# usnistgov/object-detection-yolov3

Measured on AMD Instinct MI355X. Metric: images/sec (train fwd+bwd) bs=8 416x416, higher is better.
Workload: dtype f32

## Files before the change

include/yolo3hip.h:

```cpp
#ifndef YOLO3HIP_H
#define YOLO3HIP_H

#include <math.h>
#include <stddef.h>
#include <stdint.h>

#ifdef __cplusplus
extern "C" {
#endif

#define Y3_OK 0
#define Y3_EINVAL (-1)
#define Y3_ELAUNCH (-2)

typedef void* y3_stream_t;

const char* y3_last_error(void);
int y3_debug_div(int x, int d);
int y3_version(void);

#define Y3_EPI_LRELU 1u
#define Y3_EPI_ACCUM 2u
#define Y3_CONV_X3 4u
int y3_x3_split_weights(const float* w, void* planes, int taps, int rows, int k_per_row, y3_stream_t stream);
int y3_x3_split_weights_batched(const float* arena, void* planes_arena, const int* table_dev, int nlayers, int total_blocks, y3_stream_t stream);
int y3_x3_prepare_weights_batched(const float* params, float* params_t, void* planes, void* planes_t, const int* table_dev, int nlayers,
                                  int total_tiles, y3_stream_t stream);

typedef struct y3_tensor {
    float* ptr;
    int n, h, w, c;
    int ld;
} y3_tensor;

int y3_conv2d_fwd(const y3_tensor* src, const float* wt, const float* bias, int ksize, int stride,
                  const y3_tensor* dst, unsigned flags, float alpha,
                  const float* scale, const float* shift, const y3_tensor* resid,
                  float* stats, void* workspace, size_t workspace_bytes, y3_stream_t stream);
int y3_conv2d_stats_tiles(int m, int cin, int ksize, int cout);
size_t y3_conv2d_fwd_workspace(int m, int cin, int ksize, int cout);
int y3_conv2d_stats_tiles_x(int m, int cin, int ksize, int cout, unsigned flags);
size_t y3_conv2d_fwd_workspace_x(int m, int cin, int ksize, int cout, unsigned flags);
int y3_conv2d_x3_ok(int m, int c, int ntaps, int nout);
int y3_conv2d_dgrad_x3_ok(const y3_tensor* ddst, int ksize, int stride, const y3_tensor* dsrc);
size_t y3_conv2d_plan(int m, int cin, int ksize, int cout, int* out13);
size_t y3_conv2d_plan_x(int m, int cin, int ksize, int cout, unsigned flags, int* out13);

int y3_conv2d_dgrad(const y3_tensor* ddst, const float* wt_t, int ksize, int stride,
                    const y3_tensor* dsrc, unsigned flags, void* workspace, size_t workspace_bytes,
                    y3_stream_t stream);
size_t y3_conv2d_dgrad_workspace(const y3_tensor* ddst, int ksize, int stride, const y3_tensor* dsrc);
size_t y3_conv2d_dgrad_workspace_x(const y3_tensor* ddst, int ksize, int stride, const y3_tensor* dsrc, unsigned flags);
int y3_conv2d_dgrad_bn(const y3_tensor* ddst, const float* wt_t, int ksize, int stride, const y3_tensor* dsrc,
                       unsigned flags, const y3_tensor* bn_a, float* bn_partials,
                       void* workspace, size_t workspace_bytes, y3_stream_t stream);
int y3_conv2d_dgrad_bn_tiles(const y3_tensor* ddst, int ksize, int stride, const y3_tensor* dsrc);
int y3_conv2d_dgrad_bn_tiles_x(const y3_tensor* ddst, int ksize, int stride, const y3_tensor* dsrc, unsigned flags);
size_t y3_conv2d_dgrad_plan_x(const y3_tensor* ddst, int ksize, int stride, const y3_tensor* dsrc, unsigned flags, int* out51);

int y3_conv2d_wgrad(const y3_tensor* src, const y3_tensor* ddst, int ksize, int stride,
                    float* dw, void* workspace, size_t workspace_bytes, y3_stream_t stream);
size_t y3_conv2d_wgrad_workspace(const y3_tensor* src, const y3_tensor* ddst, int ksize, int stride);
int y3_conv2d_wgrad_x(const y3_tensor* src, const y3_tensor* ddst, int ksize, int stride,
                      float* dw, unsigned flags, void* workspace, size_t workspace_bytes, y3_stream_t stream);
size_t y3_conv2d_wgrad_workspace_x(const y3_tensor* src, const y3_tensor* ddst, int ksize, int stride, unsigned flags);
int y3_conv2d_wgrad_x3_ok(int m, int cin, int ksize, int cout);
size_t y3_conv2d_wgrad_plan(int m, int cin, int ksize, int cout, int* out8);
size_t y3_conv2d_wgrad_plan_x(int m, int cin, int ksize, int cout, unsigned flags, int* out8);

int y3_transpose_weights(const float* wt, float* wt_t, int taps, int cin, int cout, y3_stream_t stream);
int y3_transpose_weights_batched(const float* params, float* params_t, const int* table_dev, int nlayers,
                                 int total_tiles, y3_stream_t stream);

int y3_bn_stats_finalize(const float* stats, int tiles, int c, int count,
                         const float* gamma, const float* beta, float eps, float momentum,
                         float* moving_mean, float* moving_var,
                         float* save_mean, float* save_rstd, float* scale, float* shift,
                         y3_stream_t stream);
int y3_bn_fold_inference(const float* gamma, const float* beta, const float* moving_mean,
                         const float* moving_var, float eps, int c, float* scale, float* shift,
                         y3_stream_t stream);
int y3_bn_fold_inference_batched(const float* params, const float* moving, float* chan, const int* table_dev,
                                 int nlayers, float eps, y3_stream_t stream);
int y3_bn_apply(const y3_tensor* a, const float* scale, const float* shift, const y3_tensor* resid,
                const y3_tensor* y, y3_stream_t stream);
int y3_bn_bwd_stats(const y3_tensor* dy, const y3_tensor* a, const y3_tensor* dres, int dres_accumulate,
                    const float* gamma, const float* save_mean, const float* save_rstd, float alpha,
                    float* dgamma, float* dbeta, float* dbias, float* coef,
                    void* workspace, size_t workspace_bytes, y3_stream_t stream);
// ... 219 lines not shown
```

object-detection-yolov3_amd/csrc/conv.hip:

```cpp
#include <stdlib.h>

#include <type_traits>
#include <utility>

#include "common.h"
#include "conv_plan.h"

template <int BM, int BN, int WM, int WN, int BK>
__global__ __launch_bounds__(64 * WM * WN) void conv_igemm_kernel(const ConvArgs p) {
    constexpr int THREADS = 64 * WM * WN;
    constexpr int LDA = BK + 4;
    constexpr int TM = BM / WM, TN = BN / WN, MB = TM / 32, NB = TN / 32;
    constexpr int KV = BK / 4;
    constexpr int A_TOTAL = BM * KV, A_LOADS = (A_TOTAL + THREADS - 1) / THREADS;
    constexpr int BN4 = BN / 4;
    constexpr int B_TOTAL = BK * BN4, B_LOADS = (B_TOTAL + THREADS - 1) / THREADS;
    static_assert(THREADS % KV == 0 && TM % 32 == 0 && TN % 32 == 0, "tile shape");

    __shared__ __attribute__((aligned(16))) float As[2][BM * LDA];
    __shared__ __attribute__((aligned(16))) float Bs[2][BK * BN];
    __shared__ float red[2][WM][BN];

    const int tid = threadIdx.x, lane = tid & 63, wave = tid >> 6;
    const int l31 = lane & 31, lh = lane >> 5;
// ... 1174 lines not shown
        for (int kw = 0; kw < ksize; ++kw) {
            const int t = kh * ksize + kw;
            p.tap_dhdw |= (unsigned long long)((kh - pbh + 1) | ((kw - pbw + 1) << 2)) << (4 * t);
        }
    p.src = src->ptr;
    p.ddst = ddst->ptr;
    p.H = src->h;
    p.W = src->w;
    p.C = src->c;
    p.src_ld = src->ld;
    p.OH = OH;
    p.OW = OW;
    p.sh = p.sw = stride;
    p.dd_ld = ddst->ld;
    p.Nout = ddst->c;
    p.K = taps * src->c;
    p.M = src->n * OH * OW;
    {
        const long long sb = (long long)src->n * src->h * src->w * src->ld * 4, db = (long long)p.M * ddst->ld * 4;
        Y3_CHECK_ARG(sb < 0x7fffffffLL && db < 0x7fffffffLL, "conv2d_wgrad: tensors of 2 GiB or more are not supported (32-bit buffer offsets)");
        p.src_bytes = (unsigned)sb;
        p.dd_bytes = (unsigned)db;
    }
    Y3_CHECK_ARG((flags & ~Y3_CONV_X3) == 0, "conv2d_wgrad: only Y3_CONV_X3 allowed in flags");
    const WgradPlan w = describe_wgrad(p.M, src->c, taps, p.Nout, flags);
    Y3_CHECK_ARG(!(flags & Y3_CONV_X3) || w.x3, "conv2d_wgrad: Y3_CONV_X3 does not take this shape (ask y3_conv2d_wgrad_x3_ok())");
    p.chunk = w.chunk;
    p.nbn = y3_cdiv(p.Nout, w.bn);
    p.ohw = OH * OW;
    p.ntaps = taps;
    p.dv_tiles = y3_make_div(w.tiles);
    p.dv_nbn = y3_make_div(p.nbn);
    p.dv_ohw = y3_make_div(p.ohw);
    p.dv_ow = y3_make_div(OW);
    const size_t need = w.ws_bytes;
    Y3_CHECK_ARG(workspace_bytes >= need && (need == 0 || workspace), "conv2d_wgrad: workspace %zu < %zu", workspace_bytes, need);
    Y3_CHECK_ARG(need < 0x7ff00000ull, "conv2d_wgrad: slab area too large (%zu bytes)", need);
    p.tickets = w.in_kernel ? (int*)workspace : nullptr;
    if (p.tickets)
        if (int e = check_tickets("conv2d_wgrad", workspace, (hipStream_t)stream)) return e;
    p.out = w.splits > 1 ? (float*)((char*)workspace + Y3_WS_HEADER) : dw;
    p.dw = dw;
    hipStream_t st = (hipStream_t)stream;
    p.tiles = w.tiles;
    p.splits = w.splits;
    dim3 grid((unsigned)w.grid);
    constexpr int pad40 = 8192;
    if (w.x3) {
// ... 41 lines not shown
```

object-detection-yolov3_amd/csrc/conv_plan.cpp:

```cpp
#include <stdlib.h>
#include "host.h"
#include "conv_plan.h"

static TileCfg pick_tile(int M, int Nout) {
    TileCfg t;
    if (Nout <= 32)
        t = {128, 32, 16};
    else if (Nout <= 64)
        t = {128, 64, 16};
    else {
        const long long t128 = (long long)y3_cdiv(M, 128) * y3_cdiv(Nout, 128);
        const long long t64x128 = (long long)y3_cdiv(M, 64) * y3_cdiv(Nout, 128);
        if (t128 >= 600)
            t = {128, 128, 16};
        else if (t64x128 >= 600)
            t = {64, 128, 16};
        else
            t = {64, 64, 16};
    }
    return t;
}
void whole_tiles(ConvPlan& pl, int chunk) {
    pl.f = pl.tiles;
    pl.s0 = pl.s1 = 1;
// ... 448 lines not shown
            w.bn = 64;
        } else if (K <= 576) {
            w.bkr = 64;
        }
    }
    w.tiles = y3_cdiv(K, w.bkr) * y3_cdiv(Nout, w.bn);
    constexpr int want_waves = 4096;
    const int waves_per_wg = (w.bkr == 64 && w.bn == 32) ? 2 : 4;
    int splits = y3_cdiv(want_waves, w.tiles * waves_per_wg);
    const int maxs = y3_cdiv(M, 128);
    if (splits > maxs) splits = maxs;
    if (splits < 1) splits = 1;
    if (splits < y3_cdiv(M, Y3_WG_TABLE - 32)) splits = y3_cdiv(M, Y3_WG_TABLE - 32);
    int chunk = y3_cdiv(M, splits);
    chunk = y3_cdiv(chunk, 32) * 32;
    w.splits = y3_cdiv(M, chunk);
    w.chunk = chunk;
    return w;
}

static bool wgrad_x3_shape_ok(int K, int Nout, int taps, int cin) {
    return cin % 4 == 0 && K >= 128 && Nout >= 128 && (taps == 1 || y3_is_pow2(cin));
}
static WgradPlan plan_wgrad_x3(int K, int Nout, int M) {
    WgradPlan w;
    w.bkr = 128;
    w.bn = 128;
    w.tiles = y3_cdiv(K, 128) * y3_cdiv(Nout, 128);
    constexpr int want = 480;
    int splits = want / w.tiles;
    if (splits < 1) splits = 1;
    if (w.tiles > 256 && splits < 3) splits = 3;
    const int maxs = y3_cdiv(M, 192);
    if (splits > maxs) splits = maxs;
    if (splits < y3_cdiv(M, Y3_WG_TABLE - 96)) splits = y3_cdiv(M, Y3_WG_TABLE - 96);
    int chunk = y3_cdiv(M, splits);
    chunk = y3_cdiv(chunk, 96) * 96;
    w.splits = y3_cdiv(M, chunk);
    w.chunk = chunk;
    return w;
}

static bool wgrad_in_kernel(const WgradPlan& w) {
    return w.splits > 1 && w.splits <= Y3_WG_FANIN && w.tiles <= Y3_MAX_TICKETS;
}
static size_t wgrad_ws_bytes(const WgradPlan& w, int K, int Nout) {
    if (w.splits <= 1) return 0;
    if (wgrad_in_kernel(w)) return (size_t)Y3_WS_HEADER + (size_t)w.tiles * w.splits * w.bkr * w.bn * sizeof(float);
    return (size_t)Y3_WS_HEADER + (size_t)w.splits * K * Nout * sizeof(float);
}
WgradPlan describe_wgrad(int M, int cin, int taps, int Nout, unsigned flags) {
    const bool x3 = (flags & Y3_CONV_X3) && wgrad_x3_shape_ok(taps * cin, Nout, taps, cin);
    WgradPlan w = x3 ? plan_wgrad_x3(taps * cin, Nout, M) : plan_wgrad(taps * cin, Nout, M, taps);
    w.x3 = x3;
    w.grid = (w.splits >= 32 ? y3_cdiv(w.splits, 8) * 8 : w.splits) * w.tiles;
    w.in_kernel = wgrad_in_kernel(w);
    w.ws_bytes = wgrad_ws_bytes(w, taps * cin, Nout);
    return w;
}

extern "C" size_t y3_conv2d_wgrad_plan(int m, int cin, int ksize, int cout, int* out8) { return y3_conv2d_wgrad_plan_x(m, cin, ksize, cout, 0u, out8); }
extern "C" size_t y3_conv2d_wgrad_plan_x(int m, int cin, int ksize, int cout, unsigned flags, int* out8) {
    const WgradPlan w = describe_wgrad(m, cin, ksize * ksize, cout, flags);
    if (out8) {
        const int v[8] = {w.bkr, w.bn, w.splits, w.chunk, w.tiles, w.in_kernel ? 1 : 0, w.grid, Y3_WG_TABLE};
        for (int i = 0; i < 8; ++i) out8[i] = v[i];
    }
    return w.ws_bytes;
}

extern "C" int y3_conv2d_wgrad_x3_ok(int m, int cin, int ksize, int cout) {
    return (m > 0 && wgrad_x3_shape_ok(ksize * ksize * cin, cout, ksize * ksize, cin)) ? 1 : 0;
}
extern "C" size_t y3_conv2d_wgrad_workspace_x(const y3_tensor* src, const y3_tensor* ddst, int ksize, int stride, unsigned flags) {
    (void)stride;
    return describe_wgrad(ddst->n * ddst->h * ddst->w, src->c, ksize * ksize, ddst->c, flags).ws_bytes;
}
extern "C" size_t y3_conv2d_wgrad_workspace(const y3_tensor* src, const y3_tensor* ddst, int ksize, int stride) {
    return y3_conv2d_wgrad_workspace_x(src, ddst, ksize, stride, 0u);
}
```

object-detection-yolov3_amd/csrc/conv_x3.hip:

```cpp
#include "conv_fast.h"

typedef __bf16 y3_bf16x8 __attribute__((ext_vector_type(8)));
typedef __bf16 y3_bf16x2 __attribute__((ext_vector_type(2)));
typedef float y3_f32x2 __attribute__((ext_vector_type(2)));

__device__ __forceinline__ unsigned x3_pk(float a, float b) {
    const y3_f32x2 v = {a, b};
    return __builtin_bit_cast(unsigned, __builtin_convertvector(v, y3_bf16x2));
}
__device__ __forceinline__ float x3_lo(unsigned pk) { return __uint_as_float(pk << 16); }
__device__ __forceinline__ float x3_hi(unsigned pk) { return __uint_as_float(pk & 0xffff0000u); }

#ifndef Y3_X3_GB
#define Y3_X3_GB 4
#endif

template <int BM, int BN, int WM, int WN, bool DENSE, bool BNS>
__device__ __forceinline__ void conv_x3_body(const FastArgs& p, const int braw, const int grid) {
    constexpr int BK = 16, KV = 4;
    constexpr int THREADS = 64 * WM * WN;
    constexpr int TM = BM / WM, TN = BN / WN, MB = TM / 32, NB = TN / 32;
    constexpr int A_LOADS = BM * KV / THREADS;
    constexpr int B_LOADS = BN * 6 / THREADS;
    static_assert((BM * KV) % THREADS == 0 && (BN * 6) % THREADS == 0 && TM % 32 == 0 && TN % 32 == 0, "tile shape");
// ... 579 lines not shown
}

template <int BM, int BN, int WM, int WN>
static void x3_launch_tile(const FastArgs& p, bool dense, int grid, hipStream_t st) {
    const dim3 g(grid), b(64 * WM * WN);
    if (p.bn_a)
        hipLaunchKernelGGL((conv_x3_kernel<BM, BN, WM, WN, true, true>), g, b, 0, st, p);
    else if (dense)
        hipLaunchKernelGGL((conv_x3_kernel<BM, BN, WM, WN, true, false>), g, b, 0, st, p);
    else
        hipLaunchKernelGGL((conv_x3_kernel<BM, BN, WM, WN, false, false>), g, b, 0, st, p);
}

typedef short y3_s16x4 __attribute__((ext_vector_type(4)));

__device__ __forceinline__ y3_bf16x8 x3_tr_pair(const unsigned short* a0, const unsigned short* a1) {
    const y3_s16x4 lo = __builtin_amdgcn_ds_read_tr16_b64_v4i16((y3_s16x4 __attribute__((address_space(3)))*)(a0));
    const y3_s16x4 hi = __builtin_amdgcn_ds_read_tr16_b64_v4i16((y3_s16x4 __attribute__((address_space(3)))*)(a1));
    typedef short s16x8 __attribute__((ext_vector_type(8)));
    const s16x8 v = {lo[0], lo[1], lo[2], lo[3], hi[0], hi[1], hi[2], hi[3]};
    return __builtin_bit_cast(y3_bf16x8, v);
}

template <int BKR, int BN, int WM, int WN>
__global__ __launch_bounds__(64 * WM * WN, 2) void conv_wgrad_x3_kernel(const WgradArgs p) {
    constexpr int BP = 16;
    constexpr int THREADS = 64 * WM * WN;
    constexpr int TM = BKR / WM, TN = BN / WN, MB = TM / 32, NB = TN / 32;
    constexpr int KR4 = BKR / 4, BN4 = BN / 4;
    static_assert(BKR == 128 && BN == 128 && THREADS == 256, "the swizzled [16][128] images and the loader are written for 128 x 128 tiles");
    constexpr int A_LOADS = BP * KR4 / THREADS, B_LOADS = BP * BN4 / THREADS;
    constexpr int PSTEP = THREADS / KR4;
    constexpr int PLANE = BP * 128;
    constexpr int OPB = 3 * PLANE;
    constexpr int BUF = 2 * OPB;
    __shared__ __attribute__((aligned(16))) unsigned short lds[2 * BUF];
    __shared__ uint2 pix[Y3_WG_TABLE];

    const int tid = threadIdx.x, lane = tid & 63, wave = tid >> 6;
    const int wm = wave / WN, wn = wave % WN;
    int splits = p.splits, tiles = p.tiles, nbn = p.nbn, chunk = p.chunk, aM = p.M, ohw = p.ohw, OW = p.OW, aH = p.H, aW = p.W;
    int src_ld = p.src_ld, csh = p.sh, csw = p.sw, ntaps = p.ntaps;
    unsigned dt_m = p.dv_tiles.mul, dn_m = p.dv_nbn.mul, dohw_m = p.dv_ohw.mul, dow_m = p.dv_ow.mul;
    int dt_s = p.dv_tiles.shift, dn_s = p.dv_nbn.shift, dohw_s = p.dv_ohw.shift, dow_s = p.dv_ow.shift;
    unsigned dhdw_lo = (unsigned)p.tap_dhdw, dhdw_hi = (unsigned)(p.tap_dhdw >> 32);
    Y3_PIN_S(splits); Y3_PIN_S(tiles); Y3_PIN_S(nbn); Y3_PIN_S(chunk); Y3_PIN_S(aM); Y3_PIN_S(ohw); Y3_PIN_S(OW); Y3_PIN_S(aH); Y3_PIN_S(aW);
    Y3_PIN_S(src_ld); Y3_PIN_S(csh); Y3_PIN_S(csw); Y3_PIN_S(ntaps);
    Y3_PIN_S(dt_m); Y3_PIN_S(dn_m); Y3_PIN_S(dohw_m); Y3_PIN_S(dow_m); Y3_PIN_S(dt_s); Y3_PIN_S(dn_s); Y3_PIN_S(dohw_s); Y3_PIN_S(dow_s);
    Y3_PIN_S(dhdw_lo); Y3_PIN_S(dhdw_hi);
    const Y3Div dv_tiles = {dt_m, dt_s}, dv_nbn = {dn_m, dn_s}, dv_ohw = {dohw_m, dohw_s}, dv_ow = {dow_m, dow_s};
    const unsigned long long tap_dhdw = ((unsigned long long)dhdw_hi << 32) | dhdw_lo;
    int split, bid;
    if (splits >= 32) {
        const int xcd = blockIdx.x & 7, jx = blockIdx.x >> 3;
        const int q = y3_div(jx, dv_tiles);
        split = q * 8 + xcd;
        bid = jx - q * tiles;
    } else {
// ... 17 lines not shown
                const int oh = y3_div(r, dv_ow), ow = r - oh * OW;
                const int ih0 = oh * csh, iw0 = ow * csw;
                off = (unsigned)(((n * aH + ih0) * aW + iw0) * src_ld) * 4u;
                for (int t = 0; t < ntaps; ++t) {
                    const int code = (int)((tap_dhdw >> (4 * t)) & 15ull);
                    const int ih = ih0 + (code & 3) - 1, iw = iw0 + (code >> 2) - 1;
                    if ((unsigned)ih < (unsigned)aH && (unsigned)iw < (unsigned)aW) msk |= 1u << t;
                }
            }
            pix[pl] = make_uint2(off, msk);
        }
    }
    const __amdgpu_buffer_rsrc_t rs_src = __builtin_amdgcn_make_buffer_rsrc(const_cast<float*>(p.src), 0, p.src_bytes, 0x00020000);
    const __amdgpu_buffer_rsrc_t rs_dd = __builtin_amdgcn_make_buffer_rsrc(const_cast<float*>(p.ddst), 0, p.dd_bytes, 0x00020000);
    const int a_kv = tid % KR4;
    const int ak = k0 + a_kv * 4;
    const bool ak_ok = ak < p.K;
    const int atap = ak_ok ? (ak >> p.logC) : 0;
    const int ac = ak & p.cmask;
    const int acode = (int)((tap_dhdw >> (4 * atap)) & 15ull);
    const int a_tapoff = ((((acode & 3) - 1) * p.W + ((acode >> 2) - 1)) * p.src_ld + ac) * 4;
    const unsigned a_bit = ak_ok ? 1u << atap : 0u;
    const int pp0 = tid / KR4;
    const int bnn = n0 + a_kv * 4;
    const bool bn_ok = bnn < p.Nout;
    const unsigned b_lane = (unsigned)(bnn * 4);
    auto swz = [](int row) { return ((row & 3) << 2) | ((row >> 2) & 3); };
    int st_off[A_LOADS];
#pragma unroll
    for (int i = 0; i < A_LOADS; ++i) {
        const int row = pp0 + i * PSTEP;
        st_off[i] = row * 128 + 8 * ((a_kv >> 1) ^ swz(row)) + 4 * (a_kv & 1);
    }
    int fr_a[MB][2], fr_b[NB][2];
    {
        const int g = lane >> 4, li = lane & 15, q = li >> 2, pc = li & 3, h = g >> 1;
#pragma unroll
        for (int j = 0; j < 2; ++j) {
            const int row = 8 * h + 4 * j + q;
#pragma unroll
            for (int i = 0; i < MB; ++i) {
                const int c = wm * TM + i * 32 + 16 * (g & 1) + 4 * pc;
                fr_a[i][j] = row * 128 + 8 * ((c >> 3) ^ swz(row)) + (c & 4);
            }
#pragma unroll
            for (int i = 0; i < NB; ++i) {
                const int c = wn * TN + i * 32 + 16 * (g & 1) + 4 * pc;
                fr_b[i][j] = row * 128 + 8 * ((c >> 3) ^ swz(row)) + (c & 4);
            }
        }
    }

    f32x4 ra[3][A_LOADS], rb[3][B_LOADS];
    uint2 pe[A_LOADS];
    auto tload = [&](int step) {
#pragma unroll
        for (int i = 0; i < A_LOADS; ++i) pe[i] = pix[step * BP + pp0 + i * PSTEP];
    };
    auto gload_a = [&](auto I, int step, auto S) {
        constexpr int i = decltype(I)::value;
        const bool ok = ((pe[i].y & a_bit) != 0) & (step < nsteps);
        ra[decltype(S)::value][i] = __builtin_amdgcn_raw_buffer_load_b128(rs_src, ok ? pe[i].x + (unsigned)a_tapoff : Y3_OOB, 0, 0);
    };
    auto gload_b = [&](auto I, int step, auto S) {
        constexpr int i = decltype(I)::value;
        const int m = mbeg + step * BP + pp0 + i * PSTEP;
        const bool ok = (m < mend) & bn_ok;
        rb[decltype(S)::value][i] = __builtin_amdgcn_raw_buffer_load_b128(rs_dd, ok ? (unsigned)(m * p.dd_ld) * 4u + b_lane : Y3_OOB, 0, 0);
    };
    X3Pk pk = {0, 0};
    auto sub = [&](auto S, auto E, int buf) {
        constexpr int set = decltype(S)::value, e = decltype(E)::value, w = e / 4, sb = e % 4;
        if constexpr (w < A_LOADS) {
            unsigned short* d = &lds[buf * BUF + st_off[w]];
            x3_split_sub<sb>(ra[set][w], pk, d, d + PLANE, d + 2 * PLANE);
        } else {
            unsigned short* d = &lds[buf * BUF + OPB + st_off[w - A_LOADS]];
            x3_split_sub<sb>(rb[set][w - A_LOADS], pk, d, d + PLANE, d + 2 * PLANE);
        }
    };
    y3_bf16x8 FA[2][3][MB], FB[2][3][NB];
    auto read_a = [&](auto F, auto PC, int i, int buf) {
        const unsigned short* b = &lds[buf * BUF + decltype(PC)::value * PLANE];
        FA[decltype(F)::value][decltype(PC)::value][i] = x3_tr_pair(b + fr_a[i][0], b + fr_a[i][1]);
    };
    auto read_b = [&](auto F, auto PC, int j, int buf) {
        const unsigned short* b = &lds[buf * BUF + OPB + decltype(PC)::value * PLANE];
        FB[decltype(F)::value][decltype(PC)::value][j] = x3_tr_pair(b + fr_b[j][0], b + fr_b[j][1]);
    };

    f32x16 acc[MB][NB];
#pragma unroll
    for (int i = 0; i < MB; ++i)
#pragma unroll
        for (int j = 0; j < NB; ++j)
#pragma unroll
            for (int r = 0; r < 16; ++r) acc[i][j][r] = 0.f;

    using C0 = std::integral_constant<int, 0>;
    using C1 = std::integral_constant<int, 1>;
    using C2 = std::integral_constant<int, 2>;
    constexpr int NW = A_LOADS + B_LOADS;
    __syncthreads();
    if (nsteps > 0) {
        constexpr int NMG = MB * NB, NM = 6 * NMG, SB = Y3_X3_GB * NMG, SP = NM - SB;
        constexpr int NR1 = NB + MB + MB, NS = NW * 4;
        constexpr int NR2 = MB + NB + NB, RS2 = (NR2 + 1) / 2;
        static_assert(NR1 <= SB && RS2 + (NW + 1) / 2 + 1 <= SP, "not enough MFMA slots for the events of a step");
        auto step = [&](auto U, int s6) {
            constexpr int u = decltype(U)::value, cur = u & 1;
            using F = std::integral_constant<int, cur>;
            using G = std::integral_constant<int, cur ^ 1>;
            using RS = std::integral_constant<int, (u + 1) % 3>;
            const int st = s6 + u;
            y3_for_each_ic(std::make_integer_sequence<int, NM>{}, [&](auto Mi) {
                constexpr int m = decltype(Mi)::value;
                constexpr int g = m / NMG, i = (m % NMG) / NB, j = m % NB;
                constexpr int pa = g < 3 ? 0 : (g < 5 ? 1 : 2), pb = g < 3 ? g : (g == 3 ? 0 : (g == 4 ? 1 : 0));
                if constexpr (m == SB) {
                    y3_lds_barrier();
                    __builtin_amdgcn_sched_barrier(0);
                }
                acc[i][j] = __builtin_amdgcn_mfma_f32_32x32x16_bf16(FA[cur][pa][i], FB[cur][pb][j], acc[i][j], 0, 0, 0);
                __builtin_amdgcn_sched_barrier(0);
                if constexpr (m < SB) {
                    if constexpr (m < NB)
                        read_b(F{}, C2{}, m, cur);
                    else if constexpr (m < NB + MB)
// ... 96 lines not shown
#pragma unroll
                    for (int r = 0; r < 4; ++r) {
                        const f32x4 v = __builtin_amdgcn_raw_buffer_load_b128(rs_slab, base2, (unsigned)(((i * NB + j) * 4 + r) * THREADS * 16), 16 );
#pragma unroll
                        for (int e = 0; e < 4; ++e) acc[i][j][4 * r + e] = z == 0 ? v[e] : acc[i][j][4 * r + e] + v[e];
                    }
        }
    }
    float* out = p.tickets != nullptr ? p.dw : p.out + (p.splits > 1 ? (long long)split * p.K * p.Nout : 0ll);
#pragma unroll
    for (int j = 0; j < NB; ++j) {
        const int n = n0 + wn * TN + j * 32 + l31;
#pragma unroll
        for (int i = 0; i < MB; ++i)
#pragma unroll
            for (int r = 0; r < 16; ++r) {
                const int k = k0 + wm * TM + i * 32 + (r & 3) + 8 * (r >> 2) + 4 * lh;
                if (k < p.K && n < p.Nout) out[(long long)k * p.Nout + n] = acc[i][j][r];
            }
    }
}

bool y3_wgrad_x3_launch(const WgradArgs& p, int bkr, int bn, unsigned grid, hipStream_t st) {
    if (bkr != 128 || bn != 128) return false;
    hipLaunchKernelGGL((conv_wgrad_x3_kernel<128, 128, 2, 2>), dim3(grid), dim3(256), 0, st, p);
    return true;
}

__device__ __forceinline__ void x3_split_store(const float* __restrict__ w, unsigned short* __restrict__ planes, long long e, int rows, int C) {
    const long long tr = e / C;
    const int c = (int)(e - tr * C);
    const long long tap = tr / rows;
    const int row = (int)(tr - tap * rows);
    f32x4 r = *reinterpret_cast<const f32x4*>(w + e);
    const unsigned a0 = x3_pk(r[0], r[1]), a1 = x3_pk(r[2], r[3]);
    r[0] -= x3_lo(a0); r[1] -= x3_hi(a0); r[2] -= x3_lo(a1); r[3] -= x3_hi(a1);
    const unsigned b0 = x3_pk(r[0], r[1]), b1 = x3_pk(r[2], r[3]);
    r[0] -= x3_lo(b0); r[1] -= x3_hi(b0); r[2] -= x3_lo(b1); r[3] -= x3_hi(b1);
    unsigned short* d = planes + (((tap * (C >> 4) + (c >> 4)) * rows + row) * 3) * 16 + (c & 15);
    *reinterpret_cast<uint2*>(d) = make_uint2(a0, a1);
    *reinterpret_cast<uint2*>(d + 16) = make_uint2(b0, b1);
    *reinterpret_cast<uint2*>(d + 32) = make_uint2(x3_pk(r[0], r[1]), x3_pk(r[2], r[3]));
}
__global__ __launch_bounds__(256) void x3_split_weights_kernel(const float* __restrict__ w, unsigned short* __restrict__ planes, long long count, int rows, int C) {
    const long long e = ((long long)blockIdx.x * 256 + threadIdx.x) * 4;
    if (e < count) x3_split_store(w, planes, e, rows, C);
}
__global__ __launch_bounds__(256) void x3_split_weights_batched_kernel(const float* __restrict__ arena, unsigned short* __restrict__ planes_arena,
// ... 126 lines not shown
```

object-detection-yolov3_amd/yolo3/_hip.py:

```python
import ctypes as C
import os

import torch

_HERE = os.path.dirname(os.path.abspath(__file__))
LIB_PATH = os.environ.get('Y3_LIB') or os.path.join(_HERE, '_lib', 'libyolo3hip.so')


class HipLibraryMissing(ImportError):
    pass


class HipError(RuntimeError):
    pass


if not os.path.exists(LIB_PATH):
    raise HipLibraryMissing(
        'libyolo3hip.so not found at %s: build it with `make -C object-detection-yolov3_amd/csrc` '
        '(hipcc --offload-arch=gfx950).  There is no CPU fallback.' % LIB_PATH)

lib = C.CDLL(LIB_PATH)


# ... 10 lines not shown
    'y3_debug_div': (i32, [i32, i32]),
    'y3_version': (i32, []),
    'y3_conv2d_fwd': (i32, [TP, fp, fp, i32, i32, TP, u32, f32, fp, fp, TP, fp, vp, sz, vp]),
    'y3_conv2d_stats_tiles': (i32, [i32, i32, i32, i32]),
    'y3_conv2d_fwd_workspace': (sz, [i32, i32, i32, i32]),
    'y3_conv2d_dgrad': (i32, [TP, fp, i32, i32, TP, u32, vp, sz, vp]),
    'y3_conv2d_stats_tiles_x': (i32, [i32, i32, i32, i32, u32]),
    'y3_conv2d_fwd_workspace_x': (sz, [i32, i32, i32, i32, u32]),
    'y3_conv2d_x3_ok': (i32, [i32, i32, i32, i32]),
    'y3_conv2d_dgrad_x3_ok': (i32, [TP, i32, i32, TP]),
    'y3_x3_split_weights': (i32, [fp, vp, i32, i32, i32, vp]),
    'y3_x3_split_weights_batched': (i32, [fp, vp, ip, i32, i32, vp]),
    'y3_x3_prepare_weights_batched': (i32, [fp, fp, vp, vp, ip, i32, i32, vp]),
    'y3_conv2d_dgrad_workspace_x': (sz, [TP, i32, i32, TP, u32]),
    'y3_conv2d_dgrad_bn_tiles_x': (i32, [TP, i32, i32, TP, u32]),
    'y3_conv2d_dgrad_workspace': (sz, [TP, i32, i32, TP]),
    'y3_conv2d_dgrad_bn': (i32, [TP, fp, i32, i32, TP, u32, TP, fp, vp, sz, vp]),
    'y3_conv2d_dgrad_bn_tiles': (i32, [TP, i32, i32, TP]),
    'y3_conv2d_wgrad': (i32, [TP, TP, i32, i32, fp, vp, sz, vp]),
    'y3_conv2d_wgrad_workspace': (sz, [TP, TP, i32, i32]),
    'y3_conv2d_wgrad_x': (i32, [TP, TP, i32, i32, fp, u32, vp, sz, vp]),
    'y3_conv2d_wgrad_workspace_x': (sz, [TP, TP, i32, i32, u32]),
    'y3_conv2d_wgrad_x3_ok': (i32, [i32, i32, i32, i32]),
    'y3_transpose_weights': (i32, [fp, fp, i32, i32, i32, vp]),
    'y3_transpose_weights_batched': (i32, [fp, fp, ip, i32, i32, vp]),
    'y3_bn_stats_finalize': (i32, [fp, i32, i32, i32, fp, fp, f32, f32, fp, fp, fp, fp, fp, fp, vp]),
    'y3_bn_fold_inference': (i32, [fp, fp, fp, fp, f32, i32, fp, fp, vp]),
    'y3_bn_fold_inference_batched': (i32, [fp, fp, fp, ip, i32, f32, vp]),
    'y3_bn_apply': (i32, [TP, fp, fp, TP, TP, vp]),
    'y3_bn_bwd_stats': (i32, [TP, TP, TP, i32, fp, fp, fp, f32, fp, fp, fp, fp, vp, sz, vp]),
    'y3_bn_bwd_workspace': (sz, [i32, i32]),
    'y3_bn_bwd_apply': (i32, [TP, TP, fp, f32, TP, vp]),
    'y3_bn_bwd_apply_fanin': (i32, [TP, TP, fp, f32, TP, TP, i32, vp]),
    'y3_bn_bwd_finalize_tiles': (i32, [fp, i32, i32, i32, fp, fp, fp, f32, fp, fp, fp, fp, vp]),
    'y3_upsample_sum2x_fwd': (i32, [TP, TP, vp]),
    'y3_upsample_sum2x_bwd': (i32, [TP, TP, vp]),
    'y3_spp_fwd': (i32, [TP, TP, vp]),
    'y3_spp_fwd_bf16': (i32, [TP, TP, vp]),
    'y3_spp_bwd': (i32, [TP, TP, TP, i32, vp]),
    'y3_copy': (i32, [TP, TP, vp]),
    'y3_conv2d_fwd_bf16': (i32, [TP, vp, fp, i32, i32, TP, i32, u32, f32, fp, fp, TP, vp]),
    'y3_conv2d_fwd_bf16_ws': (i32, [TP, vp, fp, i32, i32, TP, i32, u32, f32, fp, fp, TP, vp, sz, vp]),
    'y3_conv2d_fwd_bf16_workspace': (sz, [i32, i32, i32, i32]),
    'y3_conv2d_fwd_bf16_plan': (sz, [TP, vp, fp, i32, i32, TP, i32, u32, f32, fp, fp, TP, vp, sz, ip]),
    'y3_f32_to_bf16': (i32, [fp, vp, sz, vp]),
    'y3_conv2d_first_bf16': (i32, [TP, fp, fp, TP, u32, f32, fp, fp, vp]),
# ... 53 lines not shown
    'y3_mosaic_batch': (i32, [fp, i32, i32, i32, i32, vp, fp, vp]),
    'y3_format_labels': (i32, [ip, ip, i32, i32, C.POINTER(C.c_float), i32, i32, i32, i32, fp, fp, fp, vp]),
    'y3_eval_offsets':(i32, [ip, i32, i32, i32, ip, vp]),
    'y3_eval_match': (i32, [fp, i32, i32, i32, i32, f32, f32, ip, ip, fp, i32, i32, fp, ip, i32, i32, C.POINTER(C.c_float), i32, ip,
                            vp, vp, C.c_longlong, vp]),
    'y3_eval_ap': (i32, [vp, vp, C.c_longlong, i32, i32, ip, vp, sz, fp, fp, ip, ip, vp]),
    'y3_eval_ap_workspace_bytes': (sz, [C.c_longlong, i32]),
    'y3_eval_match_ranges': (i32, [fp, i32, i32, i32, i32, f32, f32, ip, ip, fp, i32, i32, fp, ip, i32, i32, C.POINTER(C.c_float), i32,
                                   C.POINTER(C.c_float), C.POINTER(C.c_float), i32, ip, vp, vp, vp, C.c_longlong, vp]),
    'y3_eval_ap_ranges': (i32, [vp, vp, vp, C.c_longlong, i32, i32, i32, ip, vp, sz, fp, fp, ip, ip, ip, ip, ip, fp, fp, fp, vp]),
    'y3_eval_ap_ranges_workspace_bytes': (sz, [C.c_longlong, i32, i32]),
}

for _name, (_res, _args) in SIGNATURES.items():
    _f = getattr(lib, _name)
    _f.restype = _res
    _f.argtypes = _args

EPI_LRELU = 1
EPI_ACCUM = 2
BF16_ROUTE_PP, BF16_ROUTE_C32, BF16_ROUTE_C64, BF16_ROUTE_RING = 1, 2, 3, 4
BF16_NO_PATCH = 8
CONV_X3 = 4


def check(rc, what=''):
    if rc != 0:
        raise HipError('%s failed (%d): %s' % (what or 'libyolo3hip call', rc, lib.y3_last_error().decode()))


def view(t, n, h, w, c, ld=None, offset=0):
    return Tensor(t.data_ptr() + t.element_size() * offset, n, h, w, c, c if ld is None else ld)


def float_array(vals):
    arr = (C.c_float * len(vals))(*[float(v) for v in vals])
    return arr


def int_array(vals):
    return (C.c_int * len(vals))(*[int(v) for v in vals])
```

object-detection-yolov3_amd/yolo3/model.py:

```python
import collections
import contextlib
import functools
import math
import os
import warnings

import numpy as np
import torch

from . import _hip
from . import streams
from ._hip import lib, check, view, int_array, EPI_LRELU, EPI_ACCUM, CONV_X3, BF16_NO_PATCH

BN_EPS = 1e-3
BN_MOMENTUM = 0.99
LRELU_ALPHA = 0.2
BF16_PATCH_MIN_BYTES = 300e6
ALIGN = 64


def ema_one_minus_decay(ema_decay, ema_warmup, t):
    d = float(ema_decay) * (1.0 - math.exp(-float(t) / float(ema_warmup)))
    return np.float32(1.0 - d)


BOX_LOSSES = ('mse', 'giou', 'diou', 'ciou')


def check_box_loss_args(box_loss, box_loss_weight=1.0):
    if box_loss not in BOX_LOSSES:
        raise ValueError('box_loss must be one of {}, got {!r}'.format(', '.join(BOX_LOSSES), box_loss))
    try:
        w = float(box_loss_weight)
    except (TypeError, ValueError):
        raise ValueError('box_loss_weight must be a number, got {!r}'.format(box_loss_weight))
# ... 330 lines not shown
        self.conv_ws_bytes = 0
        self._conv_ws_users = []
        if not tr:
            self._emit(self.fwd, lib.y3_bn_fold_inference_batched, P.data_ptr(), mdl.moving.data_ptr(), mdl.chan.data_ptr(),
                       mdl.fold_table().data_ptr(), mdl.fold_layers, BN_EPS)
        if tr:
            self.dz = torch.empty(max_mc, dtype=torch.float32, device=dev)
            self.bnb_ws = torch.zeros(1024 + 512 * 6 * 64 * 8, dtype=torch.uint8, device=dev)
        ptr = functools.partial(self._at, P)

        def conv_layer(src, out=None, resid=None):
            i = li[0]
            li[0] += 1
            sp = specs[i]
            oh, ow = -(-src.h // sp.s), -(-src.w // sp.s)
            y = out if out is not None else self._new(N, oh, ow, sp.cout, dtype=act)
            a = self._new(N, oh, ow, sp.cout) if tr else None
            rv = resid.v if resid is not None else None
            ch = self._at(mdl.chan, sp.ch_off)
            cs = sp.cout * 4
            scale, shift, smean, srstd, coef = ch, ch + cs, ch + 2 * cs, ch + 3 * cs, ch + 4 * cs
            x3 = _Layer(CONV_X3 if not bf and mdl.x3_forward(sp, N * oh * ow) else 0,
                        CONV_X3 if tr and src is not x0 and mdl.x3_dgrad(a.v, sp.k, sp.s, src.v) else 0,
                        CONV_X3 if tr and mdl.x3_wgrad(sp, N * oh * ow) else 0, (smean, srstd, coef))
            if x3.fwd:
                self.x3_fwd.append(i)
            wfwd = self._at(mdl.planes_t, sp.w_off) if x3.fwd else ptr(sp.w_off)
            if tr:
                tiles = lib.y3_conv2d_stats_tiles_x(a.m, sp.cin_pad, sp.k, sp.cout, x3.fwd)
                assert tiles * 2 * sp.cout <= self.stats_ws.numel()
                self._conv_call(self.fwd, lib.y3_conv2d_fwd, src.v, wfwd, ptr(sp.b_off), sp.k, sp.s, a.v, EPI_LRELU | x3.fwd,
                                LRELU_ALPHA, None, None, None, self.stats_ws.data_ptr())
                self._emit(self.fwd, lib.y3_bn_stats_finalize, self.stats_ws.data_ptr(), tiles, sp.cout, a.m, ptr(sp.g_off), ptr(sp.be_off),
                           BN_EPS, BN_MOMENTUM, self._at(mdl.moving, sp.mv_off), self._at(mdl.moving, mdl.moving_stride + sp.mv_off),
                           smean, srstd, scale, shift)
                self._emit(self.fwd, lib.y3_bn_apply, a.v, scale, shift, rv, y.v)
                self.ops.append(('conv_layer', i, src, a, y, resid, x3))
            elif bf and i > 0:
                moved = 2 * y.m * (sp.s * sp.s * sp.cin_pad + sp.cout * (2 if resid is not None else 1))
                self._conv_call(self.fwd, lib.y3_conv2d_fwd_bf16_ws, src.v, self._at(mdl.params_t_bf16, sp.w_off), ptr(sp.b_off), sp.k, sp.s, y.v, 0,
                                EPI_LRELU | (0 if moved >= BF16_PATCH_MIN_BYTES else BF16_NO_PATCH), LRELU_ALPHA, scale, shift, rv)
            elif bf and sp.cin_pad == 4 and sp.cout == 32 and sp.k == 3 and sp.s == 1:
                self._emit(self.fwd, lib.y3_conv2d_first_bf16, src.v, ptr(sp.w_off), ptr(sp.b_off), y.v, EPI_LRELU, LRELU_ALPHA, scale, shift)
            elif bf:
                y32 = self._new(N, oh, ow, sp.cout)
                self._conv_call(self.fwd, lib.y3_conv2d_fwd, src.v, ptr(sp.w_off), ptr(sp.b_off), sp.k, sp.s, y32.v, EPI_LRELU,
                                LRELU_ALPHA, scale, shift, None, None)
# ... 470 lines not shown
        self._adam_call = self._adam_launch()
        self._init_weights(seed)
        self.model = _CallableModel(self, False)
        self.model_feature_maps = _CallableModel(self, True)
        self.optimizer = self

    def x3_forward(self, sp, m_out):
        if self.conv_arithmetic == 'f32' or not lib.y3_conv2d_x3_ok(m_out, sp.cin_pad, sp.k * sp.k, sp.cout):
            return False
        return self.conv_arithmetic == 'x3-all' or sp.k == 3

    def x3_dgrad(self, ddst, k, s, dsrc):
        if self.conv_arithmetic == 'f32' or not lib.y3_conv2d_dgrad_x3_ok(ddst, k, s, dsrc):
            return False
        if self.conv_arithmetic == 'x3-all':
            return True
        if k != 3:
            return False
        if s == 2:
            return dsrc.c >= 128
        return ddst.c >= 128 and dsrc.c >= 64

    def x3_wgrad(self, sp, m_out):
        if self.conv_arithmetic == 'f32' or not lib.y3_conv2d_wgrad_x3_ok(m_out, sp.cin_pad, sp.k, sp.cout):
            return False
        return self.conv_arithmetic == 'x3-all' or sp.k == 3 or m_out >= 5000

    def _init_weights(self, seed):
        rng = np.random.default_rng(seed)
        layers = []
        for sp in self.specs:
            limit = math.sqrt(6.0 / (sp.k * sp.k * sp.cin + sp.k * sp.k * sp.cout))
            d = dict(W=rng.uniform(-limit, limit, (sp.k, sp.k, sp.cin, sp.cout)).astype(np.float32), b=np.zeros(sp.cout, np.float32))
            if sp.bn:
                d.update(gamma=np.ones(sp.cout, np.float32), beta=np.zeros(sp.cout, np.float32), mean=np.zeros(sp.cout, np.float32),
                         var=np.ones(sp.cout, np.float32))
            layers.append(d)
        self.set_weights(layers)

    def set_weights(self, layers):
        assert len(layers) == len(self.specs)
        host = np.zeros(self.arena_floats, np.float32)
        mov = np.zeros(2 * self.moving_stride, np.float32)
        mov[self.moving_stride:] = 1.0
        for sp, d in zip(self.specs, layers):
            Wk = np.asarray(d['W'], np.float32)
            assert Wk.shape == (sp.k, sp.k, sp.cin, sp.cout), (Wk.shape, (sp.k, sp.k, sp.cin, sp.cout))
            Wp = np.zeros((sp.k, sp.k, sp.cin_pad, sp.cout), np.float32)
            Wp[:, :, :sp.cin, :] = Wk
# ... 455 lines not shown
```

Before: 563.6.

## Add 128x64 x3 wgrad kernel variant for 3x3 convs with 64 output channels

Extends the split-bf16 (x3) weight-gradient kernel to handle 64-wide output tiles, with a separate B-operand swizzle, loader, and a 4x1 wave layout at three workgroups per CU. 3x3 layers with 64 output channels, which previously failed the Nout>=128 check and fell back to the f32 wgrad path, now use the MFMA-based x3 path. The split count target is raised for these smaller tiles to keep the GPU occupied, at the cost of more reduction workspace and a new swizzle pattern that must stay free of bank conflicts.

```diff
diff --git a/include/yolo3hip.h b/include/yolo3hip.h
--- a/include/yolo3hip.h
+++ b/include/yolo3hip.h
@@ -22,6 +22,7 @@
 #define Y3_EPI_LRELU 1u
 #define Y3_EPI_ACCUM 2u
 #define Y3_CONV_X3 4u
+#define Y3_CONV_X3_N64 16u
 int y3_x3_split_weights(const float* w, void* planes, int taps, int rows, int k_per_row, y3_stream_t stream);
 int y3_x3_split_weights_batched(const float* arena, void* planes_arena, const int* table_dev, int nlayers, int total_blocks, y3_stream_t stream);
 int y3_x3_prepare_weights_batched(const float* params, float* params_t, void* planes, void* planes_t, const int* table_dev, int nlayers,
@@ -65,6 +66,7 @@
                       float* dw, unsigned flags, void* workspace, size_t workspace_bytes, y3_stream_t stream);
 size_t y3_conv2d_wgrad_workspace_x(const y3_tensor* src, const y3_tensor* ddst, int ksize, int stride, unsigned flags);
 int y3_conv2d_wgrad_x3_ok(int m, int cin, int ksize, int cout);
+int y3_conv2d_wgrad_x3_n64_ok(int m, int cin, int ksize, int cout);
 size_t y3_conv2d_wgrad_plan(int m, int cin, int ksize, int cout, int* out8);
 size_t y3_conv2d_wgrad_plan_x(int m, int cin, int ksize, int cout, unsigned flags, int* out8);
 
diff --git a/object-detection-yolov3_amd/csrc/conv.hip b/object-detection-yolov3_amd/csrc/conv.hip
--- a/object-detection-yolov3_amd/csrc/conv.hip
+++ b/object-detection-yolov3_amd/csrc/conv.hip
@@ -1220,8 +1220,10 @@
         p.src_bytes = (unsigned)sb;
         p.dd_bytes = (unsigned)db;
     }
-    Y3_CHECK_ARG((flags & ~Y3_CONV_X3) == 0, "conv2d_wgrad: only Y3_CONV_X3 allowed in flags");
+    Y3_CHECK_ARG((flags & ~(Y3_CONV_X3 | Y3_CONV_X3_N64)) == 0, "conv2d_wgrad: only Y3_CONV_X3 and Y3_CONV_X3_N64 allowed in flags");
+    Y3_CHECK_ARG(!(flags & Y3_CONV_X3_N64) || (flags & Y3_CONV_X3), "conv2d_wgrad: Y3_CONV_X3_N64 goes with Y3_CONV_X3");
     const WgradPlan w = describe_wgrad(p.M, src->c, taps, p.Nout, flags);
+    Y3_CHECK_ARG(!(flags & Y3_CONV_X3_N64) || w.x3, "conv2d_wgrad: Y3_CONV_X3_N64 does not take this shape (ask y3_conv2d_wgrad_x3_n64_ok())");
     Y3_CHECK_ARG(!(flags & Y3_CONV_X3) || w.x3, "conv2d_wgrad: Y3_CONV_X3 does not take this shape (ask y3_conv2d_wgrad_x3_ok())");
     p.chunk = w.chunk;
     p.nbn = y3_cdiv(p.Nout, w.bn);
diff --git a/object-detection-yolov3_amd/csrc/conv_plan.cpp b/object-detection-yolov3_amd/csrc/conv_plan.cpp
--- a/object-detection-yolov3_amd/csrc/conv_plan.cpp
+++ b/object-detection-yolov3_amd/csrc/conv_plan.cpp
@@ -494,12 +494,15 @@
 static bool wgrad_x3_shape_ok(int K, int Nout, int taps, int cin) {
     return cin % 4 == 0 && K >= 128 && Nout >= 128 && (taps == 1 || y3_is_pow2(cin));
 }
-static WgradPlan plan_wgrad_x3(int K, int Nout, int M) {
+static bool wgrad_x3_n64_shape_ok(int Nout, int taps, int cin) {
+    return taps == 9 && Nout == 64 && cin >= 32 && y3_is_pow2(cin);
+}
+static WgradPlan plan_wgrad_x3(int K, int Nout, int M, int bn) {
     WgradPlan w;
     w.bkr = 128;
-    w.bn = 128;
-    w.tiles = y3_cdiv(K, 128) * y3_cdiv(Nout, 128);
-    constexpr int want = 480;
+    w.bn = bn;
+    w.tiles = y3_cdiv(K, 128) * y3_cdiv(Nout, bn);
+    const int want = bn == 64 ? 720 : 480;
     int splits = want / w.tiles;
     if (splits < 1) splits = 1;
     if (w.tiles > 256 && splits < 3) splits = 3;
@@ -522,8 +525,9 @@
     return (size_t)Y3_WS_HEADER + (size_t)w.splits * K * Nout * sizeof(float);
 }
 WgradPlan describe_wgrad(int M, int cin, int taps, int Nout, unsigned flags) {
-    const bool x3 = (flags & Y3_CONV_X3) && wgrad_x3_shape_ok(taps * cin, Nout, taps, cin);
-    WgradPlan w = x3 ? plan_wgrad_x3(taps * cin, Nout, M) : plan_wgrad(taps * cin, Nout, M, taps);
+    const bool n64 = (flags & Y3_CONV_X3_N64) != 0;
+    const bool x3 = (flags & Y3_CONV_X3) && (n64 ? wgrad_x3_n64_shape_ok(Nout, taps, cin) : wgrad_x3_shape_ok(taps * cin, Nout, taps, cin));
+    WgradPlan w = x3 ? plan_wgrad_x3(taps * cin, Nout, M, n64 ? 64 : 128) : plan_wgrad(taps * cin, Nout, M, taps);
     w.x3 = x3;
     w.grid = (w.splits >= 32 ? y3_cdiv(w.splits, 8) * 8 : w.splits) * w.tiles;
     w.in_kernel = wgrad_in_kernel(w);
@@ -544,6 +548,9 @@
 extern "C" int y3_conv2d_wgrad_x3_ok(int m, int cin, int ksize, int cout) {
     return (m > 0 && wgrad_x3_shape_ok(ksize * ksize * cin, cout, ksize * ksize, cin)) ? 1 : 0;
 }
+extern "C" int y3_conv2d_wgrad_x3_n64_ok(int m, int cin, int ksize, int cout) {
+    return (m > 0 && cin > 0 && wgrad_x3_n64_shape_ok(cout, ksize * ksize, cin)) ? 1 : 0;
+}
 extern "C" size_t y3_conv2d_wgrad_workspace_x(const y3_tensor* src, const y3_tensor* ddst, int ksize, int stride, unsigned flags) {
     (void)stride;
     return describe_wgrad(ddst->n * ddst->h * ddst->w, src->c, ksize * ksize, ddst->c, flags).ws_bytes;
diff --git a/object-detection-yolov3_amd/csrc/conv_x3.hip b/object-detection-yolov3_amd/csrc/conv_x3.hip
--- a/object-detection-yolov3_amd/csrc/conv_x3.hip
+++ b/object-detection-yolov3_amd/csrc/conv_x3.hip
@@ -625,18 +625,19 @@
     return __builtin_bit_cast(y3_bf16x8, v);
 }
 
-template <int BKR, int BN, int WM, int WN>
-__global__ __launch_bounds__(64 * WM * WN, 2) void conv_wgrad_x3_kernel(const WgradArgs p) {
+template <int BKR, int BN, int WM, int WN, int GB = Y3_X3_GB, int WGS = 2>
+__global__ __launch_bounds__(64 * WM * WN, WGS) void conv_wgrad_x3_kernel(const WgradArgs p) {
     constexpr int BP = 16;
     constexpr int THREADS = 64 * WM * WN;
     constexpr int TM = BKR / WM, TN = BN / WN, MB = TM / 32, NB = TN / 32;
     constexpr int KR4 = BKR / 4, BN4 = BN / 4;
-    static_assert(BKR == 128 && BN == 128 && THREADS == 256, "the swizzled [16][128] images and the loader are written for 128 x 128 tiles");
+    static_assert(BKR == 128 && (BN == 128 || BN == 64) && THREADS == 256,
+                  "the swizzled [16][128] / [16][64] images and the loaders are written for 128 x 128 and 128 x 64 tiles");
     constexpr int A_LOADS = BP * KR4 / THREADS, B_LOADS = BP * BN4 / THREADS;
-    constexpr int PSTEP = THREADS / KR4;
-    constexpr int PLANE = BP * 128;
-    constexpr int OPB = 3 * PLANE;
-    constexpr int BUF = 2 * OPB;
+    constexpr int PSTEP = THREADS / KR4, PSTEP_B = THREADS / BN4;
+    constexpr int PLANE = BP * BKR, PLANE_B = BP * BN;
+    constexpr int OPB = 3 * PLANE, OPB_B = 3 * PLANE_B;
+    constexpr int BUF = OPB + OPB_B;
     __shared__ __attribute__((aligned(16))) unsigned short lds[2 * BUF];
     __shared__ uint2 pix[Y3_WG_TABLE];
 
@@ -700,15 +701,22 @@
     const int a_tapoff = ((((acode & 3) - 1) * p.W + ((acode >> 2) - 1)) * p.src_ld + ac) * 4;
     const unsigned a_bit = ak_ok ? 1u << atap : 0u;
     const int pp0 = tid / KR4;
-    const int bnn = n0 + a_kv * 4;
+    const int b_kv = tid % BN4, bp0 = tid / BN4;
+    const int bnn = n0 + b_kv * 4;
     const bool bn_ok = bnn < p.Nout;
     const unsigned b_lane = (unsigned)(bnn * 4);
     auto swz = [](int row) { return ((row & 3) << 2) | ((row >> 2) & 3); };
-    int st_off[A_LOADS];
+    auto swz_b = [](int row) { return BN == 128 ? (((row & 3) << 2) | ((row >> 2) & 3)) : ((((row >> 1) & 1) << 2) | ((row >> 2) & 3)); };
+    int st_off[A_LOADS], st_off_b[B_LOADS];
 #pragma unroll
     for (int i = 0; i < A_LOADS; ++i) {
         const int row = pp0 + i * PSTEP;
         st_off[i] = row * 128 + 8 * ((a_kv >> 1) ^ swz(row)) + 4 * (a_kv & 1);
+    }
+#pragma unroll
+    for (int i = 0; i < B_LOADS; ++i) {
+        const int row = bp0 + i * PSTEP_B;
+        st_off_b[i] = row * BN + 8 * ((b_kv >> 1) ^ swz_b(row)) + 4 * (b_kv & 1);
     }
     int fr_a[MB][2], fr_b[NB][2];
     {
@@ -724,7 +732,7 @@
 #pragma unroll
             for (int i = 0; i < NB; ++i) {
                 const int c = wn * TN + i * 32 + 16 * (g & 1) + 4 * pc;
-                fr_b[i][j] = row * 128 + 8 * ((c >> 3) ^ swz(row)) + (c & 4);
+                fr_b[i][j] = row * BN + 8 * ((c >> 3) ^ swz_b(row)) + (c & 4);
             }
         }
     }
@@ -742,7 +750,7 @@
     };
     auto gload_b = [&](auto I, int step, auto S) {
         constexpr int i = decltype(I)::value;
-        const int m = mbeg + step * BP + pp0 + i * PSTEP;
+        const int m = mbeg + step * BP + bp0 + i * PSTEP_B;
         const bool ok = (m < mend) & bn_ok;
         rb[decltype(S)::value][i] = __builtin_amdgcn_raw_buffer_load_b128(rs_dd, ok ? (unsigned)(m * p.dd_ld) * 4u + b_lane : Y3_OOB, 0, 0);
     };
@@ -753,8 +761,8 @@
             unsigned short* d = &lds[buf * BUF + st_off[w]];
             x3_split_sub<sb>(ra[set][w], pk, d, d + PLANE, d + 2 * PLANE);
         } else {
-            unsigned short* d = &lds[buf * BUF + OPB + st_off[w - A_LOADS]];
-            x3_split_sub<sb>(rb[set][w - A_LOADS], pk, d, d + PLANE, d + 2 * PLANE);
+            unsigned short* d = &lds[buf * BUF + OPB + st_off_b[w - A_LOADS]];
+            x3_split_sub<sb>(rb[set][w - A_LOADS], pk, d, d + PLANE_B, d + 2 * PLANE_B);
         }
     };
     y3_bf16x8 FA[2][3][MB], FB[2][3][NB];
@@ -763,7 +771,7 @@
         FA[decltype(F)::value][decltype(PC)::value][i] = x3_tr_pair(b + fr_a[i][0], b + fr_a[i][1]);
     };
     auto read_b = [&](auto F, auto PC, int j, int buf) {
-        const unsigned short* b = &lds[buf * BUF + OPB + decltype(PC)::value * PLANE];
+        const unsigned short* b = &lds[buf * BUF + OPB + decltype(PC)::value * PLANE_B];
         FB[decltype(F)::value][decltype(PC)::value][j] = x3_tr_pair(b + fr_b[j][0], b + fr_b[j][1]);
     };
 
@@ -781,7 +789,7 @@
     constexpr int NW = A_LOADS + B_LOADS;
     __syncthreads();
     if (nsteps > 0) {
-        constexpr int NMG = MB * NB, NM = 6 * NMG, SB = Y3_X3_GB * NMG, SP = NM - SB;
+        constexpr int NMG = MB * NB, NM = 6 * NMG, SB = GB * NMG, SP = NM - SB;
         constexpr int NR1 = NB + MB + MB, NS = NW * 4;
         constexpr int NR2 = MB + NB + NB, RS2 = (NR2 + 1) / 2;
         static_assert(NR1 <= SB && RS2 + (NW + 1) / 2 + 1 <= SP, "not enough MFMA slots for the events of a step");
@@ -924,8 +932,12 @@
 }
 
 bool y3_wgrad_x3_launch(const WgradArgs& p, int bkr, int bn, unsigned grid, hipStream_t st) {
-    if (bkr != 128 || bn != 128) return false;
-    hipLaunchKernelGGL((conv_wgrad_x3_kernel<128, 128, 2, 2>), dim3(grid), dim3(256), 0, st, p);
+    if (bkr == 128 && bn == 128)
+        hipLaunchKernelGGL((conv_wgrad_x3_kernel<128, 128, 2, 2>), dim3(grid), dim3(256), 0, st, p);
+    else if (bkr == 128 && bn == 64)
+        hipLaunchKernelGGL((conv_wgrad_x3_kernel<128, 64, 4, 1, 3, 3>), dim3(grid), dim3(256), 0, st, p);
+    else
+        return false;
     return true;
 }
 
diff --git a/object-detection-yolov3_amd/yolo3/_hip.py b/object-detection-yolov3_amd/yolo3/_hip.py
--- a/object-detection-yolov3_amd/yolo3/_hip.py
+++ b/object-detection-yolov3_amd/yolo3/_hip.py
@@ -56,6 +56,7 @@
     'y3_conv2d_wgrad_x': (i32, [TP, TP, i32, i32, fp, u32, vp, sz, vp]),
     'y3_conv2d_wgrad_workspace_x': (sz, [TP, TP, i32, i32, u32]),
     'y3_conv2d_wgrad_x3_ok': (i32, [i32, i32, i32, i32]),
+    'y3_conv2d_wgrad_x3_n64_ok': (i32, [i32, i32, i32, i32]),
     'y3_transpose_weights': (i32, [fp, fp, i32, i32, i32, vp]),
     'y3_transpose_weights_batched': (i32, [fp, fp, ip, i32, i32, vp]),
     'y3_bn_stats_finalize': (i32, [fp, i32, i32, i32, fp, fp, f32, f32, fp, fp, fp, fp, fp, fp, vp]),
@@ -155,6 +156,7 @@
 BF16_ROUTE_PP, BF16_ROUTE_C32, BF16_ROUTE_C64, BF16_ROUTE_RING = 1, 2, 3, 4
 BF16_NO_PATCH = 8
 CONV_X3 = 4
+CONV_X3_N64 = 16
 
 
 def check(rc, what=''):
diff --git a/object-detection-yolov3_amd/yolo3/model.py b/object-detection-yolov3_amd/yolo3/model.py
--- a/object-detection-yolov3_amd/yolo3/model.py
+++ b/object-detection-yolov3_amd/yolo3/model.py
@@ -10,7 +10,7 @@
 
 from . import _hip
 from . import streams
-from ._hip import lib, check, view, int_array, EPI_LRELU, EPI_ACCUM, CONV_X3, BF16_NO_PATCH
+from ._hip import lib, check, view, int_array, EPI_LRELU, EPI_ACCUM, CONV_X3, CONV_X3_N64, BF16_NO_PATCH
 
 BN_EPS = 1e-3
 BN_MOMENTUM = 0.99
@@ -387,7 +387,7 @@
             scale, shift, smean, srstd, coef = ch, ch + cs, ch + 2 * cs, ch + 3 * cs, ch + 4 * cs
             x3 = _Layer(CONV_X3 if not bf and mdl.x3_forward(sp, N * oh * ow) else 0,
                         CONV_X3 if tr and src is not x0 and mdl.x3_dgrad(a.v, sp.k, sp.s, src.v) else 0,
-                        CONV_X3 if tr and mdl.x3_wgrad(sp, N * oh * ow) else 0, (smean, srstd, coef))
+                        mdl.x3_wgrad(sp, N * oh * ow) if tr else 0, (smean, srstd, coef))
             if x3.fwd:
                 self.x3_fwd.append(i)
             wfwd = self._at(mdl.planes_t, sp.w_off) if x3.fwd else ptr(sp.w_off)
@@ -904,9 +904,13 @@
         return ddst.c >= 128 and dsrc.c >= 64
 
     def x3_wgrad(self, sp, m_out):
-        if self.conv_arithmetic == 'f32' or not lib.y3_conv2d_wgrad_x3_ok(m_out, sp.cin_pad, sp.k, sp.cout):
-            return False
-        return self.conv_arithmetic == 'x3-all' or sp.k == 3 or m_out >= 5000
+        if self.conv_arithmetic == 'f32':
+            return 0
+        if lib.y3_conv2d_wgrad_x3_n64_ok(m_out, sp.cin_pad, sp.k, sp.cout):
+            return CONV_X3 | CONV_X3_N64
+        if not lib.y3_conv2d_wgrad_x3_ok(m_out, sp.cin_pad, sp.k, sp.cout):
+            return 0
+        return CONV_X3 if self.conv_arithmetic == 'x3-all' or sp.k == 3 or m_out >= 5000 else 0
 
     def _init_weights(self, seed):
         rng = np.random.default_rng(seed)
```

After: 568.5, median of 6. Within noise of the previous version (+0.9%).
